# junshutang/Make-It-3D

Measured on AMD Instinct MI355X. Metric: SDS train-steps/sec (NeRF render+SD U-Net fwd+bwd) @128x128, higher is better.
Workload: dtype f32 hash grid (fp32 gather, fp32 gradient contributions accumulated in 64-bit fixed point) + f16 MFMA MLP (torch.autocast semantics; the planes between gather, MLP and scatter hold the binary16 values autocast rounds them to), f16 U-Net

## Files before the change

make-it-3d_amd/csrc/field.hip:

```cpp
#include <hip/hip_runtime.h>

#include <type_traits>

#include "../../include/mi3d.h"
#include "mi3d_dev.h"
#include "lds_transpose.h"

namespace {

constexpr int kWave = 64;
constexpr int kWavesPerWG = 4;
constexpr int DIN = 32, DOUT = 4;

using f32x16 = __attribute__((ext_vector_type(16))) float;
using f32x4 = __attribute__((ext_vector_type(4))) float;
using f32x2 = __attribute__((ext_vector_type(2))) float;
using half8 = __attribute__((ext_vector_type(8))) _Float16;
using half2v = __attribute__((ext_vector_type(2))) _Float16;
using ushort8v = __attribute__((ext_vector_type(8))) unsigned short;

inline hipStream_t as_stream(void *s) { return reinterpret_cast<hipStream_t>(s); }

__device__ __forceinline__ int rowmap(int q, int h) { return (q & 3) + 8 * (q >> 2) + 4 * h; }

// ... 214 lines not shown
        } else if (blk < B::IDX) {
            const int tk = blk - B::W1T;
            v = nl < din ? w.W1[(32 * tk + kd) * din + nl] : 0.f;
        } else if (blk == B::IDX) {
            v = nl == kx ? 1.f : 0.f;
        } else {
            v = nl == kd ? 1.f : 0.f;
        }
        constexpr int per_unit = 16 / (int)sizeof(T);
        T *dst = reinterpret_cast<T *>(lds + (size_t)blk * block_bytes<P>() + ((q / per_unit) * kWave + lane) * 16);
        dst[q % per_unit] = (T)v;
    }
    for (int e = threadIdx.x; e < B::BIAS_TILES * 32; e += blockDim.x) {
        const int tile = e / 32, h = (e % 32) / 16, q = e % 16, row = rowmap(q, h);
        float v = 0.f;
        if (tile < NTH) v = w.b1[32 * tile + row];
        else if (tile < 2 * NTH) v = LAYERS == 3 ? w.b2[32 * (tile - NTH) + row] : 0.f;
        else v = row < DOUT ? w.b3[row] : 0.f;
        biasT[e] = P::round(v);
    }
}
__device__ __forceinline__ f32x16 bias_tile(const float *biasT, int tile, int h) {
    const f32x4 *src = reinterpret_cast<const f32x4 *>(biasT + (tile * 2 + h) * 16);
    f32x16 a;
#pragma unroll
    for (int c = 0; c < 4; ++c) {
        const f32x4 t = src[c];
        a[4 * c] = t[0]; a[4 * c + 1] = t[1]; a[4 * c + 2] = t[2]; a[4 * c + 3] = t[3];
    }
    return a;
}

template <bool FULL = false>
__device__ __forceinline__ void load_rows_half_g(const float *__restrict__ x, size_t row, size_t n, int h,
                                                 size_t plane_rows, uint32_t last_plane, uint32_t (&u)[8]) {
    row = row < n ? row : n - 1;
    if constexpr (FULL) {
        const uint32_t *src = reinterpret_cast<const uint32_t *>(x) + ((size_t)(8 * h) * plane_rows + row);
#pragma unroll
        for (int j = 0; j < 8; ++j) u[j] = src[(size_t)j * plane_rows];
        return;
    }
#pragma unroll
    for (int j = 0; j < 8; ++j) {
        const uint32_t pl = (uint32_t)(8 * h + j) < last_plane ? (uint32_t)(8 * h + j) : last_plane;
        u[j] = reinterpret_cast<const uint32_t *>(x)[(size_t)pl * plane_rows + row];
    }
}
__device__ __forceinline__ void load_rows_raw_g(const float *__restrict__ x, size_t row, size_t n, int h,
                                                size_t plane_rows, uint32_t din, float (&raw)[16]) {
    row = row < n ? row : n - 1;
    const uint32_t last_plane = din / 2 - 1;
    if (plane_rows == 0 && din == DIN) {
        const f32x4 *src = reinterpret_cast<const f32x4 *>(x + row * DIN + 16 * h);
#pragma unroll
        for (int c = 0; c < 4; ++c) {
            const f32x4 t = src[c];
#pragma unroll
            for (int i = 0; i < 4; ++i) raw[4 * c + i] = t[i];
        }
    } else if (plane_rows == 0) {
#pragma unroll
        for (int q = 0; q < 16; ++q) {
            const uint32_t f = (uint32_t)(16 * h + q) < din ? (uint32_t)(16 * h + q) : din - 1;
            raw[q] = x[row * din + f];
        }
    } else {
#pragma unroll
        for (int j = 0; j < 8; ++j) {
            const uint32_t pl = (uint32_t)(8 * h + j) < last_plane ? (uint32_t)(8 * h + j) : last_plane;
            const f32x2 t = *reinterpret_cast<const f32x2 *>(x + ((size_t)pl * plane_rows + row) * 2);
            raw[2 * j] = t[0];
            raw[2 * j + 1] = t[1];
        }
    }
}

template <class P, int NTH, int LAYERS, bool HP>
__global__ __launch_bounds__(kWave *kWavesPerWG, 2) void k_mlp_fwd_g(const float *__restrict__ x, uint32_t x_planes,
                                                                        uint32_t n, uint32_t din, Weights w,
                                                                        float *__restrict__ out,
                                                                        const int32_t *__restrict__ count, uint32_t n_stride) {
    using B = Blk<NTH, LAYERS>;
    using KB = typename P::KB;
    extern __shared__ __attribute__((aligned(16))) char lds[];
    float *biasT = reinterpret_cast<float *>(lds + (size_t)B::FWD_COUNT * block_bytes<P>());
    build_blocks_g<P, NTH, LAYERS>(lds, biasT, w, (int)din, B::FWD_COUNT);
    __syncthreads();
    const int lane = threadIdx.x & (kWave - 1), p = lane & 31, h = lane >> 5;
    const uint32_t wave = blockIdx.x * kWavesPerWG + threadIdx.x / kWave, n_waves = gridDim.x * kWavesPerWG;
    const uint32_t n_tiles = (n + 31) / 32;
    auto blk = [&](int b) {
        int l = lane;
        asm volatile("" : "+v"(l));
        return P::load_block(lds + (size_t)b * block_bytes<P>(), l);
    };
    auto bias = [&](int tile) {
        int hh = h;
        asm volatile("" : "+v"(hh));
        return bias_tile(biasT, tile, hh);
    };
    const uint32_t last_plane = din / 2 - 1;
    const uint32_t c_rows = count ? (uint32_t)max(*count, 0) : 0xFFFFFFFFu;
    for (uint32_t tile = wave; tile < n_tiles; tile += n_waves) {
        bool live = true;
        if (count) {
            const uint32_t s0 = (tile * 32u) % n_stride;
            if (s0 >= c_rows && s0 + 32u <= n_stride) continue;
            live = (s0 + (uint32_t)p) % n_stride < c_rows;
        }
        const size_t row = (size_t)tile * 32 + p;
        KB X;
        if constexpr (HP) {
            uint32_t u[8];
            load_rows_half_g(x, row, n, h, x_planes, last_plane, u);
            X = rows_kb_half<P>(u);
        } else {
            float raw[16];
            load_rows_raw_g(x, row, n, h, x_planes, din, raw);
            X = rows_kb<P>(raw);
        }
        KB H1[NTH], HL[NTH];
#pragma unroll
        for (int t = 0; t < NTH; ++t) {
            f32x16 acc = bias(t);
            P::mma(acc, blk(B::W1 + t), X);
            H1[t] = P::relu(acc);
        }
        if constexpr (LAYERS == 3) {
#pragma unroll
            for (int t = 0; t < NTH; ++t) {
                f32x16 acc = bias(NTH + t);
#pragma unroll
                for (int tk = 0; tk < NTH; ++tk) P::mma(acc, blk(B::W2 + t * NTH + tk), H1[tk]);
                HL[t] = P::relu(acc);
            }
        } else {
#pragma unroll
            for (int t = 0; t < NTH; ++t) HL[t] = H1[t];
        }
        f32x16 acc = bias(2 * NTH);
#pragma unroll
        for (int tk = 0; tk < NTH; ++tk) P::mma(acc, blk(B::W3 + tk), HL[tk]);
        if (row < n && h == 0 && live) {
            f32x4 o = {P::round(acc[0]), P::round(acc[1]), P::round(acc[2]), P::round(acc[3])};
            __builtin_nontemporal_store(o, reinterpret_cast<f32x4 *>(out + row * DOUT));
        }
    }
}

template <class P, int NTH, int LAYERS> constexpr int bwd_waves_per_simd() {
    return std::is_same<P, F32>::value && NTH == 2 && LAYERS == 3 ? 1 : 2;
}
template <class P, int NTH, int LAYERS, bool HP, bool FULL>
__global__ __launch_bounds__(kWave *kWavesPerWG, (bwd_waves_per_simd<P, NTH, LAYERS>())) void k_mlp_bwd_g(
    const float *x, uint32_t x_planes, const float *__restrict__ dout, uint32_t n, uint32_t din, Weights w, float *dx,
    uint32_t dx_planes, Grads g) {
    using B = Blk<NTH, LAYERS>;
    using KB = typename P::KB;
    constexpr int H = 32 * NTH;
    extern __shared__ __attribute__((aligned(16))) char lds[];
    float *biasT = reinterpret_cast<float *>(lds + (size_t)B::ALL_COUNT * block_bytes<P>());
    build_blocks_g<P, NTH, LAYERS>(lds, biasT, w, (int)din, B::ALL_COUNT);
    __syncthreads();
    const int lane = threadIdx.x & (kWave - 1), p = lane & 31, h = lane >> 5;
    const uint32_t wave = blockIdx.x * kWavesPerWG + threadIdx.x / kWave, n_waves = gridDim.x * kWavesPerWG;
    const uint32_t n_tiles = (n + 31) / 32;
    int lt = lane, ht = h;
    auto blk = [&](int b) { return P::load_block(lds + (size_t)b * block_bytes<P>(), lt); };
    auto blk_fresh = [&](int b) {
        int l = lane;
        asm volatile("" : "+v"(l));
        return P::load_block(lds + (size_t)b * block_bytes<P>(), l);
    };
    auto bias = [&](int tile) { return bias_tile(biasT, tile, ht); };
    [[maybe_unused]] mi3d_tr::lds_ptr tr_wr_d = nullptr, tr_wr_x = nullptr, tr_rd = nullptr;
    if constexpr (P::kLdsTranspose) {
        mi3d_tr::lds_ptr tile = mi3d_tr::to_lds(biasT + B::BIAS_TILES * 32) + (threadIdx.x / kWave) * mi3d_tr::kTileBytes;
        tr_wr_d = tile + mi3d_tr::write_offset_d(lane);
        tr_wr_x = tile + mi3d_tr::write_offset_x(lane);
        tr_rd = tile + mi3d_tr::read_offset(lane);
    }
    auto transpose = [&](const KB &a, int id_block) {
        if constexpr (P::kLdsTranspose) {
            KB r;
            if (id_block == B::IDX) mi3d_tr::write_tile<true>(tr_wr_x, a.v[0], a.v[1]);
            else mi3d_tr::write_tile<false>(tr_wr_d, a.v[0], a.v[1]);
            mi3d_tr::read_tile(tr_rd, r.v[0], r.v[1]);
            return r;
        } else {
            f32x16 t = splat(0.f);
            P::mma(t, a, blk_fresh(id_block));
            return P::cast(t);
        }
    };
    const uint32_t last_plane = FULL ? (uint32_t)(DIN / 2 - 1) : din / 2 - 1;

    f32x16 gW1[NTH], gW2[NTH][NTH], gW3[NTH];
    float gb1[NTH], gb2[NTH], gb3 = 0.f;
#pragma unroll
    for (int a = 0; a < NTH; ++a) {
        gW1[a] = splat(0.f); gW3[a] = splat(0.f); gb1[a] = 0.f; gb2[a] = 0.f;
#pragma unroll
        for (int b = 0; b < NTH; ++b) gW2[a][b] = splat(0.f);
    }

    float raw[HP ? 1 : 16];
    uint32_t rawh[HP ? 8 : 1];
    f32x4 dor;
    {
        const size_t r0 = (size_t)wave * 32 + p;
        if constexpr (HP) load_rows_half_g<FULL>(x, r0, n, h, x_planes, last_plane, rawh);
        else load_rows_raw_g(x, r0, n, h, x_planes, din, raw);
        dor = load_dout_raw(dout, r0, n);
    }
    for (uint32_t tile = wave; tile < n_tiles; tile += n_waves) {
        const size_t row = (size_t)tile * 32 + p;
        const bool valid = row < n;
        uint32_t xp = x_planes, dxp = dx_planes;
        asm volatile("" : "+s"(xp), "+s"(dxp), "+v"(lt), "+v"(ht));
        KB X;
        if constexpr (HP) X = rows_kb_half<P>(rawh);
        else X = rows_kb<P>(raw);
        const KB dO = dout_kb<P>(dor, valid && h == 0);
        auto prefetch = [&]() {
            if (tile + n_waves < n_tiles) {
                const size_t rn = ((size_t)tile + n_waves) * 32 + p;
                if constexpr (HP) load_rows_half_g<FULL>(x, rn, n, ht, xp, last_plane, rawh);
                else load_rows_raw_g(x, rn, n, P::kLdsTranspose ? ht : h, xp, din, raw);
                dor = load_dout_raw(dout, rn, n);
            }
        };
        constexpr bool late_prefetch = HP;
        if constexpr (!late_prefetch) prefetch();
        KB H1p[NTH], HL[NTH];
        {
            KB H1[NTH];
#pragma unroll
            for (int t = 0; t < NTH; ++t) {
                f32x16 acc = bias(t);
                P::mma(acc, blk(B::W1 + t), X);
                H1[t] = P::relu(acc);
            }
            if constexpr (LAYERS == 3) {
#pragma unroll
                for (int t = 0; t < NTH; ++t) {
                    f32x16 acc = bias(NTH + t);
#pragma unroll
                    for (int tk = 0; tk < NTH; ++tk) P::mma(acc, blk(B::W2 + t * NTH + tk), H1[tk]);
                    HL[t] = P::relu(acc);
                }
            } else {
#pragma unroll
                for (int t = 0; t < NTH; ++t) HL[t] = H1[t];
            }
#pragma unroll
            for (int t = 0; t < NTH; ++t) H1p[t] = transpose(H1[t], B::IDD);
        }
        KB dHL[NTH];
#pragma unroll
        for (int t = 0; t < NTH; ++t) {
            f32x16 acc = splat(0.f);
            P::mma_lo(acc, blk(B::W3T + t), dO);
            dHL[t] = P::masked(acc, HL[t]);
        }
        {
            KB dOp;
            if constexpr (P::kLdsTranspose) {
                dOp = transpose(dO, B::IDX);
            } else {
                f32x16 tO = splat(0.f);
                P::mma_lo(tO, dO, blk_fresh(B::IDX));
                dOp = P::cast(tO);
            }
            gb3 += P::sum(dOp);
#pragma unroll
            for (int t = 0; t < NTH; ++t) {
                const KB HLp = LAYERS == 3 ? transpose(HL[t], B::IDD) : H1p[t];
                P::mma(gW3[t], dOp, HLp);
            }
        }
        KB dH1p[NTH];
        if constexpr (LAYERS == 3) {
#pragma unroll
            for (int ti = 0; ti < NTH; ++ti) {
                const KB dHLp = transpose(dHL[ti], B::IDD);
                gb2[ti] += P::sum(dHLp);
#pragma unroll
                for (int tj = 0; tj < NTH; ++tj) P::mma(gW2[ti][tj], dHLp, H1p[tj]);
            }
#pragma unroll
            for (int t = 0; t < NTH; ++t) {
                f32x16 acc = splat(0.f);
#pragma unroll
                for (int tk = 0; tk < NTH; ++tk) P::mma(acc, dHL[tk], blk(B::W2T + t * NTH + tk));
                dH1p[t] = P::masked(acc, H1p[t]);
            }
        } else {
#pragma unroll
            for (int t = 0; t < NTH; ++t) dH1p[t] = transpose(dHL[t], B::IDD);
        }
        {
            const KB Xp = transpose(X, B::IDX);
            if constexpr (late_prefetch) prefetch();
#pragma unroll
            for (int t = 0; t < NTH; ++t) {
                gb1[t] += P::sum(dH1p[t]);
                P::mma(gW1[t], dH1p[t], Xp);
            }
        }
        {
            f32x16 acc = splat(0.f);
#pragma unroll
            for (int tk = 0; tk < NTH; ++tk) {
                const KB dH1 = LAYERS == 3 ? transpose(dH1p[tk], B::IDD) : dHL[tk];
                P::mma(acc, blk(B::W1T + tk), dH1);
            }
            const bool full = FULL || din == (uint32_t)DIN;
            if constexpr (HP) {
            if (valid) {
                uint32_t *dxh = reinterpret_cast<uint32_t *>(dx) + row;
                uint32_t pk[8];
#pragma unroll
                for (int c = 0; c < 4; ++c) {
                    pk[2 * c] = __builtin_bit_cast(uint32_t, __builtin_convertvector((f32x2){acc[4 * c], acc[4 * c + 1]}, half2v));
                    pk[2 * c + 1] = __builtin_bit_cast(uint32_t, __builtin_convertvector((f32x2){acc[4 * c + 2], acc[4 * c + 3]}, half2v));
                }
                if (FULL) {
                    uint32_t *dst = dxh + (size_t)(2 * h) * dxp;
#pragma unroll
                    for (int c = 0; c < 4; ++c) {
                        dst[(size_t)(4 * c) * dxp] = pk[2 * c];
                        dst[(size_t)(4 * c + 1) * dxp] = pk[2 * c + 1];
                    }
                } else if (full) {
#pragma unroll
                    for (int c = 0; c < 4; ++c) {
                        dxh[(size_t)(4 * c + 2 * h) * dxp] = pk[2 * c];
                        dxh[(size_t)(4 * c + 2 * h + 1) * dxp] = pk[2 * c + 1];
                    }
                } else {
#pragma unroll
                    for (int c = 0; c < 4; ++c) {
                        const uint32_t lvl = 4 * c + 2 * h;
                        if (lvl <= last_plane) dxh[(size_t)lvl * dxp] = pk[2 * c];
                        if (lvl + 1 <= last_plane) dxh[(size_t)(lvl + 1) * dxp] = pk[2 * c + 1];
                    }
                }
            }
            } else {
            if (valid && !dxp) {
                if (full) {
                    float *dst = dx + row * DIN + 4 * h;
#pragma unroll
                    for (int c = 0; c < 4; ++c) {
                        f32x4 o = {acc[4 * c], acc[4 * c + 1], acc[4 * c + 2], acc[4 * c + 3]};
                        __builtin_nontemporal_store(o, reinterpret_cast<f32x4 *>(dst + 8 * c));
                    }
                } else {
#pragma unroll
                    for (int q = 0; q < 16; ++q)
                        if ((uint32_t)rowmap(q, h) < din) dx[row * din + rowmap(q, h)] = acc[q];
                }
            } else if (valid) {
#pragma unroll
                for (int c = 0; c < 4; ++c) {
                    f32x2 a = {acc[4 * c], acc[4 * c + 1]}, b = {acc[4 * c + 2], acc[4 * c + 3]};
                    const uint32_t lvl = 4 * c + 2 * h;
                    if (lvl <= last_plane)
                        __builtin_nontemporal_store(a, reinterpret_cast<f32x2 *>(dx + ((size_t)lvl * dxp + row) * 2));
                    if (lvl + 1 <= last_plane)
                        __builtin_nontemporal_store(b, reinterpret_cast<f32x2 *>(dx + ((size_t)(lvl + 1) * dxp + row) * 2));
                }
            }
            }
        }
    }

    __syncthreads();
    float *red = reinterpret_cast<float *>(lds);
    const int OFF_W1 = 0, OFF_B1 = OFF_W1 + H * (int)din, OFF_W2 = OFF_B1 + H,
              OFF_B2 = OFF_W2 + (LAYERS == 3 ? H * H : 0), OFF_W3 = OFF_B2 + (LAYERS == 3 ? H : 0),
              OFF_B3 = OFF_W3 + DOUT * H, TOTAL = OFF_B3 + DOUT;
    for (int e = threadIdx.x; e < TOTAL; e += blockDim.x) red[e] = 0.f;
    __syncthreads();
#pragma unroll
    for (int q = 0; q < 16; ++q) {
        const int r = rowmap(q, h);
#pragma unroll
        for (int ti = 0; ti < NTH; ++ti) {
            if (p < (int)din) atomicAdd(&red[OFF_W1 + (32 * ti + r) * (int)din + p], gW1[ti][q]);
            if constexpr (LAYERS == 3) {
#pragma unroll
                for (int tj = 0; tj < NTH; ++tj) atomicAdd(&red[OFF_W2 + (32 * ti + r) * H + 32 * tj + p], gW2[ti][tj][q]);
            }
            if (r < DOUT) atomicAdd(&red[OFF_W3 + r * H + 32 * ti + p], gW3[ti][q]);
        }
    }
#pragma unroll
    for (int t = 0; t < NTH; ++t) {
        atomicAdd(&red[OFF_B1 + 32 * t + p], gb1[t]);
        if constexpr (LAYERS == 3) atomicAdd(&red[OFF_B2 + 32 * t + p], gb2[t]);
    }
    if (p < DOUT) atomicAdd(&red[OFF_B3 + p], gb3);
    __syncthreads();
    for (int e = threadIdx.x; e < TOTAL; e += blockDim.x) {
        const float v = red[e];
        float *dst = e < OFF_B1 ? g.dW1 + (e - OFF_W1)
                   : e < OFF_W2 ? g.db1 + (e - OFF_B1)
                   : e < OFF_B2 ? g.dW2 + (e - OFF_W2)
                   : e < OFF_W3 ? g.db2 + (e - OFF_B2)
                   : e < OFF_B3 ? g.dW3 + (e - OFF_W3)
                                : g.db3 + (e - OFF_B3);
        if (v != 0.f) unsafeAtomicAdd(dst, v);
    }
}

template <int NTH, int LAYERS, bool WG> constexpr int bwd2_waves_per_simd() { return WG && NTH == 2 && LAYERS == 3 ? 1 : 2; }
template <int NTH, int LAYERS, bool ROWS, bool WG>
__global__ __launch_bounds__(kWave *kWavesPerWG, (bwd2_waves_per_simd<NTH, LAYERS, WG>())) void k_mlp_bwd2_g(
    const float *__restrict__ x, const float *__restrict__ dout, const float *__restrict__ r, uint32_t n, uint32_t din,
    Weights w, float *__restrict__ grad_dout, float *gW1o, float *gW2o, float *gW3o) {
    using P = F32;
    using B = Blk<NTH, LAYERS>;
    using KB = typename P::KB;
    constexpr int H = 32 * NTH;
    constexpr int N_BLOCKS = WG ? B::ALL_COUNT : B::FWD_COUNT;
    extern __shared__ __attribute__((aligned(16))) char lds[];
    float *biasT = reinterpret_cast<float *>(lds + (size_t)N_BLOCKS * block_bytes<P>());
    build_blocks_g<P, NTH, LAYERS>(lds, biasT, w, (int)din, N_BLOCKS);
    __syncthreads();
    const int lane = threadIdx.x & (kWave - 1), p = lane & 31, h = lane >> 5;
    const uint32_t wave = blockIdx.x * kWavesPerWG + threadIdx.x / kWave, n_waves = gridDim.x * kWavesPerWG;
    const uint32_t n_tiles = (n + 31) / 32;
    int lt = lane, ht = h;
    auto blk = [&](int b) { return P::load_block(lds + (size_t)b * block_bytes<P>(), lt); };
    auto blk_fresh = [&](int b) {
        int l = lane;
        asm volatile("" : "+v"(l));
        return P::load_block(lds + (size_t)b * block_bytes<P>(), l);
    };
    auto bias = [&](int tile) { return bias_tile(biasT, tile, ht); };
    auto transpose = [&](const KB &a, int id_block) {
        f32x16 t = splat(0.f);
        P::mma(t, a, blk_fresh(id_block));
        return P::cast(t);
    };

    [[maybe_unused]] f32x16 gW1[NTH], gW2[NTH][NTH], gW3[NTH];
    if constexpr (WG) {
#pragma unroll
        for (int a = 0; a < NTH; ++a) {
            gW1[a] = splat(0.f); gW3[a] = splat(0.f);
#pragma unroll
            for (int b = 0; b < NTH; ++b) gW2[a][b] = splat(0.f);
        }
    }

    float raw[16], rawr[16];
    [[maybe_unused]] f32x4 dor;
    {
        const size_t r0 = (size_t)wave * 32 + p;
        load_rows_raw_g(x, r0, n, h, 0, din, raw);
        load_rows_raw_g(r, r0, n, h, 0, din, rawr);
        if constexpr (WG) dor = load_dout_raw(dout, r0, n);
    }
    for (uint32_t tile = wave; tile < n_tiles; tile += n_waves) {
        const size_t row = (size_t)tile * 32 + p;
        const bool valid = row < n;
        asm volatile("" : "+v"(lt), "+v"(ht));
        const KB X = rows_kb<P>(raw);
        KB R;
#pragma unroll
        for (int q = 0; q < 16; ++q) R.v[q] = valid ? rawr[q] : 0.f;
        [[maybe_unused]] KB dO;
        if constexpr (WG) dO = dout_kb<P>(dor, valid && h == 0);
        if (tile + n_waves < n_tiles) {
            const size_t rn = ((size_t)tile + n_waves) * 32 + p;
            load_rows_raw_g(x, rn, n, h, 0, din, raw);
            load_rows_raw_g(r, rn, n, h, 0, din, rawr);
            if constexpr (WG) dor = load_dout_raw(dout, rn, n);
        }
        KB H1[NTH], U1[NTH], HL[NTH], UL[NTH];
#pragma unroll
        for (int t = 0; t < NTH; ++t) {
            f32x16 acc = bias(t);
            P::mma(acc, blk(B::W1 + t), X);
            H1[t] = P::relu(acc);
            f32x16 u = splat(0.f);
            P::mma(u, blk(B::W1 + t), R);
            U1[t] = P::masked(u, H1[t]);
        }
        [[maybe_unused]] KB Rp;
        if constexpr (WG) Rp = transpose(R, B::IDX);
        if constexpr (LAYERS == 3) {
#pragma unroll
            for (int t = 0; t < NTH; ++t) {
                f32x16 acc = bias(NTH + t);
#pragma unroll
                for (int tk = 0; tk < NTH; ++tk) P::mma(acc, blk(B::W2 + t * NTH + tk), H1[tk]);
                HL[t] = P::relu(acc);
                f32x16 u = splat(0.f);
#pragma unroll
                for (int tk = 0; tk < NTH; ++tk) P::mma(u, blk(B::W2 + t * NTH + tk), U1[tk]);
                UL[t] = P::masked(u, HL[t]);
            }
        } else {
#pragma unroll
            for (int t = 0; t < NTH; ++t) { HL[t] = H1[t]; UL[t] = U1[t]; }
        }
        if constexpr (ROWS) {
            f32x16 acc = splat(0.f);
#pragma unroll
            for (int tk = 0; tk < NTH; ++tk) P::mma(acc, blk(B::W3 + tk), UL[tk]);
            if (valid && h == 0) {
                f32x4 o = {acc[0], acc[1], acc[2], acc[3]};
                __builtin_nontemporal_store(o, reinterpret_cast<f32x4 *>(grad_dout + row * DOUT));
            }
        }
        if constexpr (WG) {
            {
                f32x16 tO = splat(0.f);
                P::mma_lo(tO, dO, blk_fresh(B::IDX));
                const KB dOp = P::cast(tO);
#pragma unroll
                for (int t = 0; t < NTH; ++t) P::mma(gW3[t], dOp, transpose(UL[t], B::IDD));
            }
            KB dHL[NTH];
#pragma unroll
            for (int t = 0; t < NTH; ++t) {
// ... 39 lines not shown
        __syncthreads();
#pragma unroll
        for (int q = 0; q < 16; ++q) {
            const int rr = rowmap(q, h);
#pragma unroll
            for (int ti = 0; ti < NTH; ++ti) {
                if (p < (int)din) atomicAdd(&red[OFF_W1 + (32 * ti + rr) * (int)din + p], gW1[ti][q]);
                if constexpr (LAYERS == 3) {
#pragma unroll
                    for (int tj = 0; tj < NTH; ++tj) atomicAdd(&red[OFF_W2 + (32 * ti + rr) * H + 32 * tj + p], gW2[ti][tj][q]);
                }
                if (rr < DOUT) atomicAdd(&red[OFF_W3 + rr * H + 32 * ti + p], gW3[ti][q]);
            }
        }
        __syncthreads();
        for (int e = threadIdx.x; e < TOTAL; e += blockDim.x) {
            const float v = red[e];
            float *dst = e < OFF_W2 ? gW1o + (e - OFF_W1) : e < OFF_W3 ? gW2o + (e - OFF_W2) : gW3o + (e - OFF_W3);
            if (v != 0.f) unsafeAtomicAdd(dst, v);
        }
    }
}

struct HeadArgs {
    const float *x, *x2;
    float offs[MI3D_MAX_POINTS * 3];
    uint32_t P;
    float bound, blob_density, two_r2, inv_2eps;
};

__device__ __forceinline__ float head_gauss(const HeadArgs &a, const float *base, uint32_t p) {
    float d2 = 0.f;
#pragma unroll
    for (int d = 0; d < 3; ++d) {
        const float v = fminf(a.bound, fmaxf(-a.bound, base[d] + a.offs[p * 3 + d]));
        d2 += v * v;
    }
    return a.blob_density * expf(-d2 / a.two_r2);
}

__device__ __forceinline__ bool head_is_nan(float f) { return (__float_as_uint(f) & 0x7fffffffu) > 0x7f800000u; }

__device__ __forceinline__ void head_normal(const float s[6], float inv_2eps, float n[3], float v[3], float &c) {
    v[0] = -((s[0] - s[1]) * inv_2eps); v[1] = -((s[2] - s[3]) * inv_2eps); v[2] = -((s[4] - s[5]) * inv_2eps);
    const float ss = v[0] * v[0] + v[1] * v[1] + v[2] * v[2];
    c = fminf(1e32f, fmaxf(1e-20f, ss));
    const float r = 1.0f / sqrtf(c);
#pragma unroll
    for (int d = 0; d < 3; ++d) {
        float t = v[d] * r;
        if (t != t || head_is_nan(ss)) t = 0.f;
        else if (t > 3.4028234663852886e38f) t = 3.4028234663852886e38f;
        else if (t < -3.4028234663852886e38f) t = -3.4028234663852886e38f;
        n[d] = t;
    }
}

__global__ void k_head_forward(const float4 *__restrict__ h, HeadArgs a, uint32_t n, float *__restrict__ sigma,
                               float *__restrict__ albedo, float *__restrict__ normal, float *__restrict__ normal2,
                               const int32_t *__restrict__ count) {
    const uint32_t s = blockIdx.x * blockDim.x + threadIdx.x;
    if (s >= n || (count && (int32_t)s >= *count)) return;
    float bx[3] = {a.x[(size_t)s * 3], a.x[(size_t)s * 3 + 1], a.x[(size_t)s * 3 + 2]};
    const float4 h0 = h[s];
    sigma[s] = expf(h0.x + head_gauss(a, bx, 0));
    albedo[(size_t)s * 3] = 1.0f / (1.0f + expf(-h0.y));
    albedo[(size_t)s * 3 + 1] = 1.0f / (1.0f + expf(-h0.z));
    albedo[(size_t)s * 3 + 2] = 1.0f / (1.0f + expf(-h0.w));
    float sg[6], nn[3], v[3], c;
#pragma unroll
    for (uint32_t p = 0; p < 6; ++p) sg[p] = expf(h[(size_t)(1 + p) * n + s].x + head_gauss(a, bx, 1 + p));
    head_normal(sg, a.inv_2eps, nn, v, c);
    normal[(size_t)s * 3] = nn[0]; normal[(size_t)s * 3 + 1] = nn[1]; normal[(size_t)s * 3 + 2] = nn[2];
    if (a.P == 13) {
        float b2[3] = {a.x2[(size_t)s * 3], a.x2[(size_t)s * 3 + 1], a.x2[(size_t)s * 3 + 2]};
#pragma unroll
        for (uint32_t p = 0; p < 6; ++p) sg[p] = expf(h[(size_t)(7 + p) * n + s].x + head_gauss(a, b2, 7 + p));
        head_normal(sg, a.inv_2eps, nn, v, c);
        normal2[(size_t)s * 3] = nn[0]; normal2[(size_t)s * 3 + 1] = nn[1]; normal2[(size_t)s * 3 + 2] = nn[2];
    }
}

__device__ __forceinline__ void head_normal_backward(const float u[6], float inv_2eps, const float dn_in[3], float du[6]) {
    float sg[6], nn[3], v[3], c;
#pragma unroll
    for (int p = 0; p < 6; ++p) sg[p] = expf(u[p]);
    head_normal(sg, inv_2eps, nn, v, c);
    const float ss = v[0] * v[0] + v[1] * v[1] + v[2] * v[2];
    const float r = 1.0f / sqrtf(c);
    float dn[3];
#pragma unroll
    for (int d = 0; d < 3; ++d) {
        const float t = v[d] * r;
        dn[d] = (t == t && fabsf(t) <= 3.4028234663852886e38f) ? dn_in[d] : 0.f;
    }
    const float dot = dn[0] * v[0] + dn[1] * v[1] + dn[2] * v[2];
    const bool inside = ss >= 1e-20f && ss <= 1e32f;
    const float k = inside ? dot * (r / c) : 0.f;
#pragma unroll
    for (int d = 0; d < 3; ++d) {
        const float dv = head_is_nan(ss) ? ss : r * dn[d] - k * v[d];
        const float dg = -dv * inv_2eps;
        du[2 * d] = dg * expf(fminf(u[2 * d], 15.0f));
        du[2 * d + 1] = -dg * expf(fminf(u[2 * d + 1], 15.0f));
    }
}

__global__ void k_head_backward(const float4 *__restrict__ h, HeadArgs a, uint32_t n, uint32_t P_active,
                                const float *__restrict__ dsigma, const float *__restrict__ dalbedo,
                                const float *__restrict__ dnormal, const float *__restrict__ dnormal2,
                                float4 *__restrict__ dh) {
    const uint32_t s = blockIdx.x * blockDim.x + threadIdx.x;
    if (s >= n) return;
    float bx[3] = {a.x[(size_t)s * 3], a.x[(size_t)s * 3 + 1], a.x[(size_t)s * 3 + 2]};
    const float4 h0 = h[s];
    float4 g0;
    g0.x = (dsigma ? dsigma[s] : 0.f) * expf(fminf(h0.x + head_gauss(a, bx, 0), 15.0f));
    const float a0 = 1.0f / (1.0f + expf(-h0.y)), a1 = 1.0f / (1.0f + expf(-h0.z)), a2 = 1.0f / (1.0f + expf(-h0.w));
    g0.y = dalbedo ? dalbedo[(size_t)s * 3] * a0 * (1.0f - a0) : 0.f;
    g0.z = dalbedo ? dalbedo[(size_t)s * 3 + 1] * a1 * (1.0f - a1) : 0.f;
    g0.w = dalbedo ? dalbedo[(size_t)s * 3 + 2] * a2 * (1.0f - a2) : 0.f;
    dh[s] = g0;
    if (P_active < 7) return;
    float u[6], du[6], dn[3];
#pragma unroll
    for (uint32_t p = 0; p < 6; ++p) u[p] = h[(size_t)(1 + p) * n + s].x + head_gauss(a, bx, 1 + p);
#pragma unroll
    for (int d = 0; d < 3; ++d) dn[d] = dnormal ? dnormal[(size_t)s * 3 + d] : 0.f;
    head_normal_backward(u, a.inv_2eps, dn, du);
#pragma unroll
    for (uint32_t p = 0; p < 6; ++p) dh[(size_t)(1 + p) * n + s] = make_float4(du[p], 0.f, 0.f, 0.f);
    if (a.P == 13 && P_active == 13) {
        float b2[3] = {a.x2[(size_t)s * 3], a.x2[(size_t)s * 3 + 1], a.x2[(size_t)s * 3 + 2]};
#pragma unroll
        for (uint32_t p = 0; p < 6; ++p) u[p] = h[(size_t)(7 + p) * n + s].x + head_gauss(a, b2, 7 + p);
#pragma unroll
        for (int d = 0; d < 3; ++d) dn[d] = dnormal2 ? dnormal2[(size_t)s * 3 + d] : 0.f;
        head_normal_backward(u, a.inv_2eps, dn, du);
#pragma unroll
        for (uint32_t p = 0; p < 6; ++p) dh[(size_t)(7 + p) * n + s] = make_float4(du[p], 0.f, 0.f, 0.f);
    }
}

HeadArgs make_head_args(const float *x, const float *x2, const float *offsets_host, uint32_t P, float bound,
                        float blob_density, float blob_radius, float epsilon) {
    HeadArgs a;
    a.x = x; a.x2 = x2; a.P = P; a.bound = bound; a.blob_density = blob_density;
    a.two_r2 = (float)(2.0 * (double)blob_radius * (double)blob_radius);
    a.inv_2eps = 0.5f / epsilon;
    for (uint32_t i = 0; i < MI3D_MAX_POINTS * 3; ++i) a.offs[i] = i < P * 3 ? offsets_host[i] : 0.f;
    return a;
}

template <class P> constexpr size_t lds_bytes_g(int n_blocks, int bias_tiles, bool transposes = false) {
    return (size_t)n_blocks * block_bytes<P>() + (size_t)bias_tiles * 32 * sizeof(float) +
           (transposes && P::kLdsTranspose ? (size_t)kWavesPerWG * mi3d_tr::kTileBytes : 0u);
}

int grid_for(uint32_t n, int wgs_per_cu) {
    const uint32_t tiles = (n + 31) / 32, wgs = (tiles + kWavesPerWG - 1) / kWavesPerWG;
    const uint32_t cap = 256 * (uint32_t)wgs_per_cu;
    return (int)(wgs < cap ? (wgs ? wgs : 1) : cap);
}

constexpr int kBwd2WgsPerCU = 2;

bool dims_ok(uint32_t di, uint32_t dh, uint32_t dout, uint32_t layers) {
    return di >= 2 && di <= (uint32_t)DIN && di % 2 == 0 && (dh == 32 || dh == 64) && dout == DOUT &&
           (layers == 2 || layers == 3);
}

template <class P, int NTH, int LAYERS, bool HP>
void launch_fwd(dim3 grid, hipStream_t st, const float *x, uint32_t x_planes, uint32_t n, uint32_t din, const Weights &w,
                float *out, const int32_t *count, uint32_t n_stride) {
    using B = Blk<NTH, LAYERS>;
    hipLaunchKernelGGL((k_mlp_fwd_g<P, NTH, LAYERS, HP>), grid, dim3(kWave * kWavesPerWG),
                       lds_bytes_g<P>(B::FWD_COUNT, B::BIAS_TILES), st, x, x_planes, n, din, w, out, count, n_stride);
}
template <class P, int NTH, int LAYERS, bool HP>
void launch_bwd(dim3 grid, hipStream_t st, const float *x, uint32_t x_planes, const float *dout, uint32_t n, uint32_t din,
                const Weights &w, float *dx, uint32_t dx_planes, const Grads &g) {
    using B = Blk<NTH, LAYERS>;
    if (HP && din == (uint32_t)DIN)
        hipLaunchKernelGGL((k_mlp_bwd_g<P, NTH, LAYERS, HP, HP>), grid, dim3(kWave * kWavesPerWG),
                           lds_bytes_g<P>(B::ALL_COUNT, B::BIAS_TILES, true), st, x, x_planes, dout, n, din, w, dx, dx_planes, g);
    else
        hipLaunchKernelGGL((k_mlp_bwd_g<P, NTH, LAYERS, HP, false>), grid, dim3(kWave * kWavesPerWG),
                           lds_bytes_g<P>(B::ALL_COUNT, B::BIAS_TILES, true), st, x, x_planes, dout, n, din, w, dx, dx_planes, g);
}
template <class, int NTH, int LAYERS, bool>
void launch_bwd2(dim3 grid, hipStream_t st, const float *x, const float *dout, const float *r, uint32_t n, uint32_t din,
                 const Weights &w, float *grad_dout, float *gW1, float *gW2, float *gW3) {
    using B = Blk<NTH, LAYERS>;
    const dim3 block(kWave * kWavesPerWG);
    const size_t lds_all = lds_bytes_g<F32>(B::ALL_COUNT, B::BIAS_TILES), lds_fwd = lds_bytes_g<F32>(B::FWD_COUNT, B::BIAS_TILES);
    if (grad_dout && gW1)
        hipLaunchKernelGGL((k_mlp_bwd2_g<NTH, LAYERS, true, true>), grid, block, lds_all, st, x, dout, r, n, din, w, grad_dout, gW1, gW2, gW3);
    else if (gW1)
        hipLaunchKernelGGL((k_mlp_bwd2_g<NTH, LAYERS, false, true>), grid, block, lds_all, st, x, dout, r, n, din, w, grad_dout, gW1, gW2, gW3);
    else
        hipLaunchKernelGGL((k_mlp_bwd2_g<NTH, LAYERS, true, false>), grid, block, lds_fwd, st, x, dout, r, n, din, w, grad_dout, gW1, gW2, gW3);
}
#define MI3D_MLP_DISPATCH(FN, P, HP, nth, layers, ...)                     \
    do {                                                                   \
        if ((nth) == 2 && (layers) == 3) FN<P, 2, 3, HP>(__VA_ARGS__);     \
        else if ((nth) == 2) FN<P, 2, 2, HP>(__VA_ARGS__);                 \
        else if ((layers) == 3) FN<P, 1, 3, HP>(__VA_ARGS__);              \
        else FN<P, 1, 2, HP>(__VA_ARGS__);                                 \
    } while (0)

}

extern "C" {

int mi3d_mlp_supported(uint32_t dim_in, uint32_t dim_hidden, uint32_t dim_out, uint32_t num_layers) {
    return dims_ok(dim_in, dim_hidden, dim_out, num_layers) ? 1 : 0;
}

int mi3d_mlp_forward(const void *xv, uint32_t x_plane_rows, int planes_half, uint32_t n, const float *W1, const float *b1, const float *W2, const float *b2,
                     const float *W3, const float *b3, uint32_t dim_in, uint32_t dim_hidden, uint32_t dim_out,
                     int half_mode, float *out, void *stream) {
    return mi3d_mlp_forward_counted(xv, x_plane_rows, planes_half, n, nullptr, n ? n : 1u, W1, b1, W2, b2, W3, b3, dim_in,
                                    dim_hidden, dim_out, half_mode, out, stream);
}

int mi3d_mlp_forward_counted(const void *xv, uint32_t x_plane_rows, int planes_half, uint32_t n, const int32_t *count,
                             uint32_t n_stride, const float *W1, const float *b1, const float *W2, const float *b2,
                             const float *W3, const float *b3, uint32_t dim_in, uint32_t dim_hidden, uint32_t dim_out,
                             int half_mode, float *out, void *stream) {
    if (n_stride == 0) return (int)hipErrorInvalidValue;
    const uint32_t layers = (W2 == nullptr && b2 == nullptr) ? 2u : 3u;
    if (!dims_ok(dim_in, dim_hidden, dim_out, layers) || (x_plane_rows != 0 && x_plane_rows < n) ||
        (planes_half && (x_plane_rows == 0 || !half_mode)) || W1 == nullptr || b1 == nullptr || W3 == nullptr ||
        b3 == nullptr || (layers == 3 && (W2 == nullptr || b2 == nullptr)))
        return (int)hipErrorInvalidValue;
    if (n == 0) return 0;
    const float *x = reinterpret_cast<const float *>(xv);
    const Weights w{W1, b1, W2, b2, W3, b3};
    const int nth = (int)dim_hidden / 32;
    hipStream_t st = as_stream(stream);
    const dim3 grid(grid_for(n, MI3D_TUNE(MI3D_T_MLP_FWD_WGS_PER_CU, 5)));
    if (half_mode && planes_half) MI3D_MLP_DISPATCH(launch_fwd, F16, true, nth, layers, grid, st, x, x_plane_rows, n, dim_in, w, out, count, n_stride);
    else if (half_mode) MI3D_MLP_DISPATCH(launch_fwd, F16, false, nth, layers, grid, st, x, x_plane_rows, n, dim_in, w, out, count, n_stride);
    else MI3D_MLP_DISPATCH(launch_fwd, F32, false, nth, layers, grid, st, x, x_plane_rows, n, dim_in, w, out, count, n_stride);
    return (int)hipGetLastError();
}

int mi3d_mlp_backward(const void *xv, uint32_t x_plane_rows, int planes_half, const float *dout, uint32_t n, const float *W1, const float *b1,
                      const float *W2, const float *b2, const float *W3, const float *b3, uint32_t dim_in,
                      uint32_t dim_hidden, uint32_t dim_out, int half_mode, void *dxv, uint32_t dx_plane_rows, float *dW1, float *db1, float *dW2, float *db2, float *dW3, float *db3,
                      void *stream) {
    const uint32_t layers = (W2 == nullptr && b2 == nullptr) ? 2u : 3u;
    if (!dims_ok(dim_in, dim_hidden, dim_out, layers) || (x_plane_rows != 0 && x_plane_rows < n) ||
        (dx_plane_rows != 0 && dx_plane_rows < n) ||
        (planes_half && (x_plane_rows == 0 || dx_plane_rows == 0 || !half_mode)) || W1 == nullptr || b1 == nullptr ||
        W3 == nullptr || b3 == nullptr || dW1 == nullptr || db1 == nullptr || dW3 == nullptr || db3 == nullptr ||
        (layers == 3 && (W2 == nullptr || b2 == nullptr || dW2 == nullptr || db2 == nullptr)))
        return (int)hipErrorInvalidValue;
    if (dxv == xv && dx_plane_rows != x_plane_rows) return (int)hipErrorInvalidValue;
    if (n == 0) return 0;
    const float *x = reinterpret_cast<const float *>(xv);
    float *dx = reinterpret_cast<float *>(dxv);
    const Weights w{W1, b1, W2, b2, W3, b3};
    const Grads g{dW1, db1, dW2, db2, dW3, db3};
    const int nth = (int)dim_hidden / 32;
    const dim3 grid(grid_for(n, MI3D_TUNE(MI3D_T_MLP_WGS_PER_CU, 2)));
    hipStream_t st = as_stream(stream);
    if (half_mode && planes_half)
        MI3D_MLP_DISPATCH(launch_bwd, F16, true, nth, layers, grid, st, x, x_plane_rows, dout, n, dim_in, w, dx, dx_plane_rows, g);
    else if (half_mode)
        MI3D_MLP_DISPATCH(launch_bwd, F16, false, nth, layers, grid, st, x, x_plane_rows, dout, n, dim_in, w, dx, dx_plane_rows, g);
    else
        MI3D_MLP_DISPATCH(launch_bwd, F32, false, nth, layers, grid, st, x, x_plane_rows, dout, n, dim_in, w, dx, dx_plane_rows, g);
    return (int)hipGetLastError();
}

int mi3d_mlp_backward_backward(const float *x, const float *dout, const float *r, uint32_t n, const float *W1, const float *b1,
                               const float *W2, const float *b2, const float *W3, const float *b3, uint32_t dim_in,
                               uint32_t dim_hidden, uint32_t dim_out, float *grad_dout, float *gW1, float *gW2, float *gW3,
                               void *stream) {
    const uint32_t layers = (W2 == nullptr && b2 == nullptr) ? 2u : 3u;
    if (!dims_ok(dim_in, dim_hidden, dim_out, layers) || x == nullptr || dout == nullptr || r == nullptr || W1 == nullptr ||
        b1 == nullptr || W3 == nullptr || b3 == nullptr || (layers == 3 && (W2 == nullptr || b2 == nullptr)))
        return (int)hipErrorInvalidValue;
    const bool any_w = gW1 != nullptr || gW3 != nullptr || (layers == 3 && gW2 != nullptr);
    const bool all_w = gW1 != nullptr && gW3 != nullptr && (layers == 2 || gW2 != nullptr);
    if ((any_w && !all_w) || (!any_w && grad_dout == nullptr)) return (int)hipErrorInvalidValue;
    if (n == 0) return 0;
    const Weights w{W1, b1, W2, b2, W3, b3};
    const int nth = (int)dim_hidden / 32;
    const dim3 grid(grid_for(n, kBwd2WgsPerCU));
    MI3D_MLP_DISPATCH(launch_bwd2, F32, false, nth, layers, grid, as_stream(stream), x, dout, r, n, dim_in, w, grad_dout,
                      all_w ? gW1 : nullptr, gW2, gW3);
    return (int)hipGetLastError();
}

int mi3d_field_head_forward(const float *h, const float *x, const float *x2, uint32_t n, const float *offsets_host,
                            uint32_t P, float bound, float blob_density, float blob_radius, float epsilon, float *sigma,
                            float *albedo, float *normal, float *normal2, void *stream) {
    return mi3d_field_head_forward_counted(h, x, x2, n, nullptr, offsets_host, P, bound, blob_density, blob_radius, epsilon,
                                           sigma, albedo, normal, normal2, stream);
}

int mi3d_field_head_forward_counted(const float *h, const float *x, const float *x2, uint32_t n, const int32_t *count,
                                    const float *offsets_host, uint32_t P, float bound, float blob_density,
                                    float blob_radius, float epsilon, float *sigma, float *albedo, float *normal,
                                    float *normal2, void *stream) {
    if ((P != 7 && P != 13) || (P == 13 && (x2 == nullptr || normal2 == nullptr))) return (int)hipErrorInvalidValue;
    if (n == 0) return 0;
    const HeadArgs a = make_head_args(x, x2, offsets_host, P, bound, blob_density, blob_radius, epsilon);
    hipLaunchKernelGGL(k_head_forward, dim3((n + 255) / 256), dim3(256), 0, as_stream(stream),
                       reinterpret_cast<const float4 *>(h), a, n, sigma, albedo, normal, normal2, count);
    return (int)hipGetLastError();
}

int mi3d_field_head_backward(const float *h, const float *x, const float *x2, uint32_t n, const float *offsets_host,
                             uint32_t P, uint32_t P_active, float bound, float blob_density, float blob_radius,
                             float epsilon, const float *dsigma, const float *dalbedo, const float *dnormal,
                             const float *dnormal2, float *dh, void *stream) {
    if ((P != 7 && P != 13) || (P == 13 && x2 == nullptr)) return (int)hipErrorInvalidValue;
    if ((P_active != 1 && P_active != 7 && P_active != 13) || P_active > P) return (int)hipErrorInvalidValue;
    if (n == 0) return 0;
    const HeadArgs a = make_head_args(x, x2, offsets_host, P, bound, blob_density, blob_radius, epsilon);
    hipLaunchKernelGGL(k_head_backward, dim3((n + 255) / 256), dim3(256), 0, as_stream(stream),
                       reinterpret_cast<const float4 *>(h), a, n, P_active, dsigma, dalbedo, dnormal, dnormal2,
                       reinterpret_cast<float4 *>(dh));
    return (int)hipGetLastError();
}

}
```

make-it-3d_amd/csrc/mi3d_common.h:

```cpp
#pragma once
#include <math.h>
#include <stdint.h>

#if defined(__HIPCC__)
#define MI3D_HD __host__ __device__ __forceinline__
#else
#define MI3D_HD static inline
#endif

namespace mi3d {

constexpr float kSqrt3 = 1.7320508075688772f;
constexpr float kRPi = 0.3183098861837907f;

MI3D_HD float clampf(float x, float lo, float hi) { return fminf(hi, fmaxf(lo, x)); }

MI3D_HD uint32_t expand_bits(uint32_t v) {
    v = (v * 0x00010001u) & 0xFF0000FFu;
    v = (v * 0x00000101u) & 0x0F00F00Fu;
    v = (v * 0x00000011u) & 0xC30C30C3u;
    v = (v * 0x00000005u) & 0x49249249u;
    return v;
}
MI3D_HD uint32_t morton3d(uint32_t x, uint32_t y, uint32_t z) {
// ... 53 lines not shown
}

MI3D_HD int voxel_coord(float p, float mip_rbound, const MarchGrid &g) {
    const float u = fmaf(p, mip_rbound, 1.0f);
    if (g.h_pow2) return (int)clampf(u * g.half_H, 0.0f, g.Hm1);
    const double v = 0.5 * (double)u * (double)g.H;
    return (int)clampf((float)v, 0.0f, g.Hm1);
}

MI3D_HD bool march_step(const MarchRay &r, const MarchGrid &g, float &t, float &x, float &y, float &z, float &dt) {
    x = clampf(fmaf(t, r.dx, r.ox), -g.bound, g.bound);
    y = clampf(fmaf(t, r.dy, r.oy), -g.bound, g.bound);
    z = clampf(fmaf(t, r.dz, r.oz), -g.bound, g.bound);
    dt = clampf(t * g.dt_gamma, g.dt_min, g.dt_max);

    int level = 0;
    float mip_bound = g.mip_bound0, mip_rbound = g.mip_rbound0;
    if (!g.one_level) {
        const float mx = fmaxf(fabsf(x), fmaxf(fabsf(y), fabsf(z)));
        int lp = frexp_exponent(mx);
        int ld = g.h_pow2 ? frexp_exponent(dt * g.half_H) : frexp_exponent((float)((double)(dt * g.Hf) * 0.5));
        lp = lp < 0 ? 0 : lp; ld = ld < 0 ? 0 : ld;
        level = lp > ld ? lp : ld;
        level = level > g.C - 1 ? g.C - 1 : level;
        mip_bound = fminf(scalbnf(1.0f, level), g.bound);
        mip_rbound = 1.0f / mip_bound;
    }
    const int nx = voxel_coord(x, mip_rbound, g);
    const int ny = voxel_coord(y, mip_rbound, g);
    const int nz = voxel_coord(z, mip_rbound, g);

    const uint32_t index = (uint32_t)((float)level * g.H3 + (float)morton3d((uint32_t)nx, (uint32_t)ny, (uint32_t)nz));
    const bool occ = (g.bits[index >> 3] >> (index & 7u)) & 1u;
    if (occ) {
        t += dt;
        return true;
    }
    const float tx = fmaf(((float)nx + r.sx) * g.rH * 2.0f - 1.0f, mip_bound, -x) * r.rdx;
    const float ty = fmaf(((float)ny + r.sy) * g.rH * 2.0f - 1.0f, mip_bound, -y) * r.rdy;
    const float tz = fmaf(((float)nz + r.sz) * g.rH * 2.0f - 1.0f, mip_bound, -z) * r.rdz;
    const float tt = t + fmaxf(0.0f, fminf(tx, fminf(ty, tz)));
    do {
        t += clampf(t * g.dt_gamma, g.dt_min, g.dt_max);
    } while (t < tt);
    return false;
}

MI3D_HD float march_t0(float near, float noise, const MarchGrid &g) {
    return fmaf(clampf(near * g.dt_gamma, g.dt_min, g.dt_max), noise, near);
}

constexpr uint32_t kPrimeY = 2654435761u, kPrimeZ = 805459861u;

struct GridLevel {
    float scale;
    uint32_t res;
    uint32_t offset;
    uint32_t size;
    uint32_t hashed;
    uint32_t dims;
};

MI3D_HD uint32_t grid_entry(const GridLevel &L, uint32_t px, uint32_t py, uint32_t pz) {
    uint32_t index;
    if (L.hashed) {
        index = px ^ (py * kPrimeY) ^ (pz * kPrimeZ);
        index = ((L.size & (L.size - 1u)) == 0u) ? (index & (L.size - 1u)) : (index % L.size);
    } else {
        index = px;
        if (L.dims > 1) index += py * L.res;
        if (L.dims > 2) index += pz * L.res * L.res;
        if (index >= L.size) {
            index -= L.size;
            if (index >= L.size) index %= L.size;
        }
    }
    return index;
}

MI3D_HD void grid_cell(float x, float scale, uint32_t &cell, float &w) {
    const float p = fmaf(scale, x, 0.5f);
    const float fl = floorf(p);
    cell = (uint32_t)(int)fl;
    w = p - fl;
}

MI3D_HD void corner_weights(float fx, float fy, float fz, float (&w)[8]) {
    const float gx = 1.0f - fx, gy = 1.0f - fy, gz = 1.0f - fz;
    const float w00 = gx * gy, w10 = fx * gy, w01 = gx * fy, w11 = fx * fy;
    w[0] = w00 * gz; w[1] = w10 * gz; w[2] = w01 * gz; w[3] = w11 * gz;
    w[4] = w00 * fz; w[5] = w10 * fz; w[6] = w01 * fz; w[7] = w11 * fz;
}

MI3D_HD unsigned long long fixed_point(float x) {
    const double d = (double)x + 6755399441055744.0;
    return (unsigned long long)(__builtin_bit_cast(long long, d) - 0x4338000000000000ll);
}

struct GatherScale {
    float scale;
    double unscale;
};
MI3D_HD GatherScale gather_scale(float tmax) {
    int ex;
    (void)frexpf(tmax, &ex);
    int k2 = 40 - ex;
    k2 = k2 > 126 ? 126 : (k2 < -126 ? -126 : k2);
    return GatherScale{ldexpf(1.0f, k2), ldexp(1.0, -k2)};
}

MI3D_HD uint32_t merge_slot(uint32_t e) { return (e * 2654435761u) >> (32 - 9); }

MI3D_HD uint32_t face_k1(uint32_t axis, uint32_t j) {
    const uint32_t lo = j & 1u, hi = j >> 1;
    return axis == 0 ? (1u | (lo << 1) | (hi << 2)) : (axis == 1 ? (lo | 2u | (hi << 2)) : (lo | (hi << 1) | 4u));
}
MI3D_HD uint32_t face_k0(uint32_t axis, uint32_t j) { return face_k1(axis, j) & ~(1u << axis); }
MI3D_HD uint32_t face_far_coord(uint32_t axis, uint32_t j, uint32_t d, uint32_t base_d, uint32_t far_c) {
    const uint32_t lo = j & 1u, hi = j >> 1;
    if (d == axis) return far_c;
    return base_d + (d == 0 ? lo : (d == 2 ? hi : (axis == 0 ? lo : hi)));
}

struct Row12 { uint32_t w0, w1, w2; };
constexpr float kFix23 = 8388608.0f, kUnfix23 = 1.0f / 8388608.0f;
MI3D_HD uint32_t fix23(float v) {
    const uint32_t q = (uint32_t)(v * kFix23 + 0.5f);
    return q < 8388607u ? q : 8388607u;
}
MI3D_HD uint32_t pair_flip_t(uint32_t cx) {
    uint32_t t = 1;
    while (cx & 1u) { cx >>= 1; ++t; }
    return t;
}
MI3D_HD Row12 pack_row12(uint32_t e_local, uint32_t t, float w, float fx, uint32_t raw_pair) {
    const uint32_t wq = fix23(w), fq = fix23(fx);
    return Row12{e_local | (t << 13) | ((wq >> 16) << 18) | ((fq >> 16) << 25), raw_pair, (wq & 0xFFFFu) | ((fq & 0xFFFFu) << 16)};
}
MI3D_HD void unpack_row12_fields(uint32_t w0, uint32_t w2, uint32_t &e_local, uint32_t &t, float &w, float &fx) {
    e_local = w0 & 8191u;
    t = (w0 >> 13) & 31u;
    w = (float)((((w0 >> 18) & 127u) << 16) | (w2 & 0xFFFFu)) * kUnfix23;
    fx = (float)(((w0 >> 25) << 16) | (w2 >> 16)) * kUnfix23;
}

constexpr int kTrRowBytes = 72;
MI3D_HD uint32_t tr_write_offset_d(int lane) { return (uint32_t)(kTrRowBytes * (lane & 31) + 8 * (lane >> 5)); }
MI3D_HD uint32_t tr_write_offset_x(int lane) { return (uint32_t)(kTrRowBytes * (lane & 31) + 32 * (lane >> 5)); }
MI3D_HD uint32_t tr_read_offset(int lane) {
    const int t = lane & 15, g = lane >> 4;
    return (uint32_t)(kTrRowBytes * (4 * (lane >> 5) + (t >> 2)) + 8 * (4 * (g & 1) + (t & 3)));
}

}
```

Baseline: 11.00.

## Ping-pong MLP backward waves in 8-wave workgroups with phase-offset barriers

For backward MLP configurations that run two waves per SIMD, the kernel now launches 8-wave workgroups. The two halves are offset by one barrier segment, and every tile is split into two segments by s_barrier. This staggers the two wave groups on each SIMD so that one half's MFMA-heavy phase lines up with the other half's memory and transpose phase. Grid sizing moves into a shared helper that counts waves per CU, and the per-wave transpose LDS scratch now scales with waves per workgroup. The scheme adds barrier stalls and depends on every wave agreeing on trip counts; waves with no tiles are padded with zero loads.

```diff
diff --git a/make-it-3d_amd/csrc/field.hip b/make-it-3d_amd/csrc/field.hip
--- a/make-it-3d_amd/csrc/field.hip
+++ b/make-it-3d_amd/csrc/field.hip
@@ -390,8 +390,11 @@
 template <class P, int NTH, int LAYERS> constexpr int bwd_waves_per_simd() {
     return std::is_same<P, F32>::value && NTH == 2 && LAYERS == 3 ? 1 : 2;
 }
+template <class P, int NTH, int LAYERS> constexpr int bwd_waves_per_wg() {
+    return bwd_waves_per_simd<P, NTH, LAYERS>() == 2 ? (int)mi3d::kMlpPairWaves : kWavesPerWG;
+}
 template <class P, int NTH, int LAYERS, bool HP, bool FULL>
-__global__ __launch_bounds__(kWave *kWavesPerWG, (bwd_waves_per_simd<P, NTH, LAYERS>())) void k_mlp_bwd_g(
+__global__ __launch_bounds__(kWave *(bwd_waves_per_wg<P, NTH, LAYERS>()), 1) void k_mlp_bwd_g(
     const float *x, uint32_t x_planes, const float *__restrict__ dout, uint32_t n, uint32_t din, Weights w, float *dx,
     uint32_t dx_planes, Grads g) {
     using B = Blk<NTH, LAYERS>;
@@ -402,8 +405,20 @@
     build_blocks_g<P, NTH, LAYERS>(lds, biasT, w, (int)din, B::ALL_COUNT);
     __syncthreads();
     const int lane = threadIdx.x & (kWave - 1), p = lane & 31, h = lane >> 5;
-    const uint32_t wave = blockIdx.x * kWavesPerWG + threadIdx.x / kWave, n_waves = gridDim.x * kWavesPerWG;
-    const uint32_t n_tiles = (n + 31) / 32;
+    constexpr int WPW = bwd_waves_per_wg<P, NTH, LAYERS>();
+    constexpr bool PAIRED = WPW == (int)mi3d::kMlpPairWaves;
+    const uint32_t wave_in_wg = (uint32_t)__builtin_amdgcn_readfirstlane((int)(threadIdx.x / kWave));
+    const uint32_t wave = blockIdx.x * WPW + wave_in_wg, n_waves = gridDim.x * WPW;
+    const uint32_t n_tiles = mi3d::mlp_tiles(n);
+    const uint32_t trips = PAIRED ? mi3d::mlp_pair_trips(blockIdx.x, gridDim.x, n) : 0u;
+    static_assert(mi3d::kMlpPairSegments == 2, "two pair_barrier() calls per tile below");
+    auto pair_barrier = [&]() {
+        if constexpr (PAIRED) {
+            __builtin_amdgcn_sched_barrier(0);
+            __builtin_amdgcn_s_barrier();
+            __builtin_amdgcn_sched_barrier(0);
+        }
+    };
     int lt = lane, ht = h;
     auto blk = [&](int b) { return P::load_block(lds + (size_t)b * block_bytes<P>(), lt); };
     auto blk_fresh = [&](int b) {
@@ -414,7 +429,7 @@
     auto bias = [&](int tile) { return bias_tile(biasT, tile, ht); };
     [[maybe_unused]] mi3d_tr::lds_ptr tr_wr_d = nullptr, tr_wr_x = nullptr, tr_rd = nullptr;
     if constexpr (P::kLdsTranspose) {
-        mi3d_tr::lds_ptr tile = mi3d_tr::to_lds(biasT + B::BIAS_TILES * 32) + (threadIdx.x / kWave) * mi3d_tr::kTileBytes;
+        mi3d_tr::lds_ptr tile = mi3d_tr::to_lds(biasT + B::BIAS_TILES * 32) + wave_in_wg * mi3d_tr::kTileBytes;
         tr_wr_d = tile + mi3d_tr::write_offset_d(lane);
         tr_wr_x = tile + mi3d_tr::write_offset_x(lane);
         tr_rd = tile + mi3d_tr::read_offset(lane);
@@ -446,13 +461,21 @@
     float raw[HP ? 1 : 16];
     uint32_t rawh[HP ? 8 : 1];
     f32x4 dor;
-    {
+    if (wave < n_tiles) {
         const size_t r0 = (size_t)wave * 32 + p;
         if constexpr (HP) load_rows_half_g<FULL>(x, r0, n, h, x_planes, last_plane, rawh);
         else load_rows_raw_g(x, r0, n, h, x_planes, din, raw);
         dor = load_dout_raw(dout, r0, n);
-    }
-    for (uint32_t tile = wave; tile < n_tiles; tile += n_waves) {
+    } else {
+#pragma unroll
+        for (float &v : raw) v = 0.f;
+#pragma unroll
+        for (uint32_t &v : rawh) v = 0u;
+        dor = f32x4{0.f, 0.f, 0.f, 0.f};
+    }
+    for (uint32_t b = mi3d::mlp_pair_lead_barriers(wave_in_wg); PAIRED && b; --b) pair_barrier();
+    uint32_t tile = wave;
+    for (uint32_t trip = 0; PAIRED ? trip < trips : tile < n_tiles; ++trip, tile += n_waves) {
         const size_t row = (size_t)tile * 32 + p;
         const bool valid = row < n;
         uint32_t xp = x_planes, dxp = dx_planes;
@@ -518,6 +541,7 @@
                 P::mma(gW3[t], dOp, HLp);
             }
         }
+        pair_barrier();
         KB dH1p[NTH];
         if constexpr (LAYERS == 3) {
 #pragma unroll
@@ -613,7 +637,9 @@
             }
             }
         }
-    }
+        pair_barrier();
+    }
+    for (uint32_t b = mi3d::mlp_pair_tail_barriers(wave_in_wg); PAIRED && b; --b) pair_barrier();
 
     __syncthreads();
     float *red = reinterpret_cast<float *>(lds);
@@ -959,9 +985,9 @@
     return a;
 }
 
-template <class P> constexpr size_t lds_bytes_g(int n_blocks, int bias_tiles, bool transposes = false) {
+template <class P> constexpr size_t lds_bytes_g(int n_blocks, int bias_tiles, int transposing_waves = 0) {
     return (size_t)n_blocks * block_bytes<P>() + (size_t)bias_tiles * 32 * sizeof(float) +
-           (transposes && P::kLdsTranspose ? (size_t)kWavesPerWG * mi3d_tr::kTileBytes : 0u);
+           (P::kLdsTranspose ? (size_t)transposing_waves * mi3d_tr::kTileBytes : 0u);
 }
 
 int grid_for(uint32_t n, int wgs_per_cu) {
@@ -985,15 +1011,16 @@
                        lds_bytes_g<P>(B::FWD_COUNT, B::BIAS_TILES), st, x, x_planes, n, din, w, out, count, n_stride);
 }
 template <class P, int NTH, int LAYERS, bool HP>
-void launch_bwd(dim3 grid, hipStream_t st, const float *x, uint32_t x_planes, const float *dout, uint32_t n, uint32_t din,
+void launch_bwd(uint32_t waves_per_cu, hipStream_t st, const float *x, uint32_t x_planes, const float *dout, uint32_t n, uint32_t din,
                 const Weights &w, float *dx, uint32_t dx_planes, const Grads &g) {
     using B = Blk<NTH, LAYERS>;
+    constexpr int WPW = bwd_waves_per_wg<P, NTH, LAYERS>();
+    const dim3 grid(mi3d::mlp_grid(n, WPW, waves_per_cu)), block(kWave * WPW);
+    const size_t lds = lds_bytes_g<P>(B::ALL_COUNT, B::BIAS_TILES, WPW);
     if (HP && din == (uint32_t)DIN)
-        hipLaunchKernelGGL((k_mlp_bwd_g<P, NTH, LAYERS, HP, HP>), grid, dim3(kWave * kWavesPerWG),
-                           lds_bytes_g<P>(B::ALL_COUNT, B::BIAS_TILES, true), st, x, x_planes, dout, n, din, w, dx, dx_planes, g);
+        hipLaunchKernelGGL((k_mlp_bwd_g<P, NTH, LAYERS, HP, HP>), grid, block, lds, st, x, x_planes, dout, n, din, w, dx, dx_planes, g);
     else
-        hipLaunchKernelGGL((k_mlp_bwd_g<P, NTH, LAYERS, HP, false>), grid, dim3(kWave * kWavesPerWG),
-                           lds_bytes_g<P>(B::ALL_COUNT, B::BIAS_TILES, true), st, x, x_planes, dout, n, din, w, dx, dx_planes, g);
+        hipLaunchKernelGGL((k_mlp_bwd_g<P, NTH, LAYERS, HP, false>), grid, block, lds, st, x, x_planes, dout, n, din, w, dx, dx_planes, g);
 }
 template <class, int NTH, int LAYERS, bool>
 void launch_bwd2(dim3 grid, hipStream_t st, const float *x, const float *dout, const float *r, uint32_t n, uint32_t din,
@@ -1071,14 +1098,14 @@
     const Weights w{W1, b1, W2, b2, W3, b3};
     const Grads g{dW1, db1, dW2, db2, dW3, db3};
     const int nth = (int)dim_hidden / 32;
-    const dim3 grid(grid_for(n, MI3D_TUNE(MI3D_T_MLP_WGS_PER_CU, 2)));
+    const uint32_t waves_per_cu = (uint32_t)kWavesPerWG * (uint32_t)MI3D_TUNE(MI3D_T_MLP_WGS_PER_CU, 2);
     hipStream_t st = as_stream(stream);
     if (half_mode && planes_half)
-        MI3D_MLP_DISPATCH(launch_bwd, F16, true, nth, layers, grid, st, x, x_plane_rows, dout, n, dim_in, w, dx, dx_plane_rows, g);
+        MI3D_MLP_DISPATCH(launch_bwd, F16, true, nth, layers, waves_per_cu, st, x, x_plane_rows, dout, n, dim_in, w, dx, dx_plane_rows, g);
     else if (half_mode)
-        MI3D_MLP_DISPATCH(launch_bwd, F16, false, nth, layers, grid, st, x, x_plane_rows, dout, n, dim_in, w, dx, dx_plane_rows, g);
+        MI3D_MLP_DISPATCH(launch_bwd, F16, false, nth, layers, waves_per_cu, st, x, x_plane_rows, dout, n, dim_in, w, dx, dx_plane_rows, g);
     else
-        MI3D_MLP_DISPATCH(launch_bwd, F32, false, nth, layers, grid, st, x, x_plane_rows, dout, n, dim_in, w, dx, dx_plane_rows, g);
+        MI3D_MLP_DISPATCH(launch_bwd, F32, false, nth, layers, waves_per_cu, st, x, x_plane_rows, dout, n, dim_in, w, dx, dx_plane_rows, g);
     return (int)hipGetLastError();
 }
 
diff --git a/make-it-3d_amd/csrc/mi3d_common.h b/make-it-3d_amd/csrc/mi3d_common.h
--- a/make-it-3d_amd/csrc/mi3d_common.h
+++ b/make-it-3d_amd/csrc/mi3d_common.h
@@ -229,4 +229,24 @@
     return (uint32_t)(kTrRowBytes * (4 * (lane >> 5) + (t >> 2)) + 8 * (4 * (g & 1) + (t & 3)));
 }
 
-}
+constexpr uint32_t kMlpPairWaves = 8, kMlpPairSegments = 2, kMlpWavesInFlight = 2048;
+MI3D_HD uint32_t mlp_tiles(uint32_t n) { return n / 32u + (n % 32u ? 1u : 0u); }
+MI3D_HD uint32_t mlp_grid(uint32_t n, uint32_t waves_per_wg, uint32_t waves_per_cu) {
+    const uint32_t tiles = mlp_tiles(n), wgs = tiles / waves_per_wg + (tiles % waves_per_wg ? 1u : 0u);
+    const uint32_t cap = 256u * waves_per_cu / waves_per_wg;
+    return wgs < cap ? (wgs ? wgs : 1u) : (cap ? cap : 1u);
+}
+MI3D_HD uint32_t mlp_wave_trips(uint32_t wave, uint32_t n_waves, uint32_t n) {
+    const uint32_t tiles = mlp_tiles(n);
+    return wave < tiles ? (tiles - wave + n_waves - 1u) / n_waves : 0u;
+}
+MI3D_HD uint32_t mlp_pair_trips(uint32_t wg, uint32_t wgs, uint32_t n) {
+    return mlp_wave_trips(wg * kMlpPairWaves, wgs * kMlpPairWaves, n);
+}
+MI3D_HD uint32_t mlp_pair_lead_barriers(uint32_t wave_in_wg) { return wave_in_wg >= kMlpPairWaves / 2 ? kMlpPairSegments / 2 : 0u; }
+MI3D_HD uint32_t mlp_pair_tail_barriers(uint32_t wave_in_wg) { return kMlpPairSegments / 2 - mlp_pair_lead_barriers(wave_in_wg); }
+MI3D_HD uint32_t mlp_pair_barriers(uint32_t wave_in_wg, uint32_t trips) {
+    return mlp_pair_lead_barriers(wave_in_wg) + trips * kMlpPairSegments + mlp_pair_tail_barriers(wave_in_wg);
+}
+
+}
```

New measurement: 10.74. 2.4% lower.
